# PhilippBongartz/RepeatResolver

Measured on AMD Instinct MI355X. Metric: sum-of-pairs DP cells/sec, higher is better.
Workload: dtype u32

## Files before the change

### repeatresolver_amd/csrc/pwr_device.hip

```cpp
#include <hip/hip_runtime.h>

#include <algorithm>
#include <chrono>
#include <cstdint>
#include <cstdio>
#include <cstdlib>
#include <cstring>
#include <new>
#include <thread>
#include <type_traits>
#include <vector>

#include "pwr.h"

#define PWR_INF 0x40000000u
#define PWR_BIG 0x7fffffff

struct Hdr {
    int W;
    int nslots;
    int nfree;
    int cur;
    int status;
    int stop;
// ... 593 lines not shown
            const unsigned upc = (y == 0 || y == W - 1) ? PWR_INF : max(w[5], covl);
            const int gq = (int)(carry + gin);
            rec2[2 * i] = make_int4((int)w[0] - gq, (int)w[1] - gq, (int)w[2] - gq, (int)w[3] - gq);
            rec2[2 * i + 1] = make_int4((int)(upc == PWR_INF ? PWR_INF - 1u : upc) - gq, gq, (int)PWR_INF - gq, 0);
            maxS = max(maxS, max(max(w[0], w[1]), max(max(w[2], w[3]), max(w[4], w[5]))));
        }
        carry += tot;
        __syncthreads();
    }
    const unsigned mx = (unsigned)(~block_min_u32<GATHER_NT>(~maxS, sh));
    for (int o = 32; o > 0; o >>= 1) ucost += __shfl_xor(ucost, o);
    if ((tid & 63) == 0) s_u[tid >> 6] = ucost;
    __syncthreads();
    if (tid == 0) {
        unsigned long long U = 0;
        for (int w = 0; w < GATHER_NT / 64; ++w) U += s_u[w];
        __hip_atomic_store(&part[g].ucost, U, __ATOMIC_RELAXED, __HIP_MEMORY_SCOPE_AGENT);
        __hip_atomic_store(&part[g].maxS, mx, __ATOMIC_RELAXED, __HIP_MEMORY_SCOPE_AGENT);
        __hip_atomic_store(&part[g].lastcov, tag, __ATOMIC_RELEASE, __HIP_MEMORY_SCOPE_AGENT);
    }
    if (g == GATHER_G - 1 && tid < 64) {
        unsigned long long Ut = 0, cs = 0;
        unsigned mxt = 0;
        if (tid < GATHER_G) {
            while (__hip_atomic_load(&part[tid].lastcov, __ATOMIC_ACQUIRE, __HIP_MEMORY_SCOPE_AGENT) != tag) __builtin_amdgcn_s_sleep(1);
            Ut = __hip_atomic_load(&part[tid].ucost, __ATOMIC_RELAXED, __HIP_MEMORY_SCOPE_AGENT);
            mxt = __hip_atomic_load(&part[tid].maxS, __ATOMIC_RELAXED, __HIP_MEMORY_SCOPE_AGENT);
            cs = part[tid].cells;
        }
        for (int o = 32; o > 0; o >>= 1) { Ut += __shfl_xor(Ut, o); cs += __shfl_xor(cs, o); mxt = max(mxt, (unsigned)__shfl_xor((int)mxt, o)); }
        if (tid == 0) {
            const unsigned long long bound = Ut + (unsigned long long)mxt * (unsigned long long)(2 * B + 4096);
            m->maxS = mxt; m->cells = cs;
            m->wide = (jb.force64 || !(bound < (unsigned long long)PWR_INF && carry < (1u << 29))) ? 1 : 0;
            if (m->wide) st.hdr->need64 = 65;
        }
    }
}

#define V2_D 128
#define V2_PD 512
#define V2_R 64
#define V2_SPINS 256
#define FBIG 0x3fffffff
#define UNI(v) __builtin_amdgcn_readfirstlane(v)

__device__ __forceinline__ unsigned acc_push(unsigned acc, unsigned long long mask)
{
    unsigned long long carry_out;
    asm("v_addc_co_u32_e64 %0, %1, %0, %0, %2" : "+v"(acc), "=s"(carry_out) : "s"(mask));
    return acc;
}
#define ICMP_SGE 39
#define ICMP_SLE 41

#define V2_LOAD(MSX, SLOT, AU, AG, AI, GL)                                                       \
    {                                                                                            \
        _Pragma("unroll") for (int i = 0; i < C; ++i) {                                          \
            const int y_ = lo + (MSX) * MS + lc + i;                                             \
            int4 p_ = make_int4(PWR_BIG / 2, PWR_BIG / 2, PWR_BIG / 2, PWR_BIG / 2);             \
            int4 q_ = make_int4(PWR_BIG / 2, 0, PWR_BIG / 2, 0);                                 \
            if (y_ <= hi) { p_ = rec2[2 * (y_ - lo)]; q_ = rec2[2 * (y_ - lo) + 1]; }            \
            ldsS[wave][SLOT][0][lc + i] = p_.x; ldsS[wave][SLOT][1][lc + i] = p_.y;              \
            ldsS[wave][SLOT][2][lc + i] = p_.z; ldsS[wave][SLOT][3][lc + i] = p_.w;              \
            AU[i] = q_.x; AG[i] = q_.y; AI[i] = q_.z;                                            \
        }                                                                                        \
        const int yq_ = lo + (MSX) * MS - 1;                                                     \
        GL = (yq_ >= lo && yq_ <= hi) ? UNI(rec2[2 * (yq_ - lo) + 1].y) : 0;                     \
    }

template <int NW, int C>
__global__ __launch_bounds__(NW * 64) void k_fill_v2(DState st, JobBufs jb)
{
    constexpr int MS = 64 * C, RS = NW * MS;
    constexpr int MBDUMP = NW * V2_D, PTDUMP = V2_PD;
    __shared__ unsigned long long mbQ[2 * (MBDUMP + NW * 64)];
    __shared__ unsigned long long ptQ[PTDUMP + NW * 64];
    __shared__ __attribute__((aligned(16))) int ldsS[NW][2][4][MS];
    __shared__ int rdone[NW];
    __shared__ int s_done;
#define LD64(REF) __hip_atomic_load(&(REF), __ATOMIC_RELAXED, __HIP_MEMORY_SCOPE_WORKGROUP)
#define LD32LO(REF) __hip_atomic_load((unsigned *)&(REF), __ATOMIC_RELAXED, __HIP_MEMORY_SCOPE_WORKGROUP)
#define ST64(REF, VAL, TAG) __hip_atomic_store(&(REF), ((unsigned long long)(unsigned)(TAG) << 32) | (unsigned)(VAL), __ATOMIC_RELAXED, __HIP_MEMORY_SCOPE_WORKGROUP)
#define MBP(W_, X_) mbQ[2 * ((W_) * V2_D + ((X_) & (V2_D - 1)))]
#define MBM(W_, X_) mbQ[2 * ((W_) * V2_D + ((X_) & (V2_D - 1))) + 1]
#define PTB(X_) ptQ[(X_) & (V2_PD - 1)]

    const int job = blockIdx.x, tid = threadIdx.x, lane = tid & 63;
    const int wave = UNI(tid >> 6);
    JobMeta *m = &jb.meta[job];
    const int L = UNI(m->L);
    if (jb.gate_v2 && st.hdr->fallback <= 0) return;
    if (!m->active || L <= 0 || !m->ok || m->wide || NOT_MINE(jb, job)) return;
    const unsigned long long t_clk0 = __builtin_amdgcn_s_memtime(), t_real0 = __builtin_amdgcn_s_memrealtime();
    for (int i = tid; i < 2 * (MBDUMP + NW * 64); i += NW * 64) mbQ[i] = 0;
    for (int i = tid; i < PTDUMP + NW * 64; i += NW * 64) ptQ[i] = 0;
    if (tid < NW) rdone[tid] = 0;
    if (tid == 0) s_done = 0;
    __syncthreads();

    const int lo = UNI(m->lo), hi = UNI(m->hi), W = UNI(m->W), B = st.B, H = st.H;
    const int *way = jb.way + (size_t)job * jb.Lmax;
    const uint8_t *seq = st.seq + st.rowoff[UNI(m->k)];
    const int4 *rec2 = jb.rec2 + (size_t)job * jb.colcap * 2;
    uint32_t *dirs = jb.dirs + (size_t)job * jb.dirstride;
    unsigned *lastM = jb.lastM + (size_t)job * jb.NC;
// ... 291 lines not shown
                    Mprev[i] = (rel0 + i < 0) ? PWR_INF : (unsigned)(gg[i] + p);
                }
            } else {
                unsigned Mn[C];
                unsigned fa = 0;
#pragma unroll
                for (int i = 0; i < C; ++i) {
                    fa |= (tg[i] >= p) ? (1u << i) : 0u;
                    p = min(p, tg[i]);
                    Mn[i] = (rel0 + i < 0) ? PWR_INF : (unsigned)(gg[i] + p);
                }
                const unsigned mrow = needP ? ePy : PWR_INF;
                const unsigned left0 = (unsigned)__builtin_amdgcn_update_dpp((int)mrow, (int)Mn[C - 1], DPP_WAVE_SHR1, 0xF, 0xF, false);
#pragma unroll
                for (int i = 0; i < C; ++i) {
                    const unsigned lf = i ? Mn[i > 0 ? i - 1 : 0] : left0;
                    const bool inb = (unsigned)(rel0 + i) < (unsigned)Bx;
                    accA[i] = (accA[i] << 1) | ((((fa >> i) & 1u) || (inb && Mn[i] == lf)) ? 1u : 0u);
                    lastM[wave * MS + lc + i] = inb ? Mn[i] : 0xffffffffu;
                    Mprev[i] = Mn[i];
                }
            }
            nacc = (x & 15) + 1;
            if (lane == 63) {
                ST64(MBP(wave, x), P_end, x + 1);
                ST64(MBM(wave, x), Mprev[C - 1], x + 1);
                if (ms == ms_hi) ST64(PTB(x), P_end, x + 1);
            }
            ran_prev = 1;
            V2_NEXT_ROW()
        }
        if (lane == 0) __hip_atomic_store(&rdone[wave], round + 1, __ATOMIC_RELAXED, __HIP_MEMORY_SCOPE_WORKGROUP);
        __syncthreads();
        if (UNI(__hip_atomic_load(&s_done, __ATOMIC_RELAXED, __HIP_MEMORY_SCOPE_WORKGROUP)) >= NW) break;
    }
    if (round >= max_rounds) {
        if (tid == 0) { m->ok = 0; atomicCAS(&st.hdr->status, 0, PWR_ERR_INTERNAL); }
        return;
    }
    if (tid == 0) {
        m->clk = (unsigned)(__builtin_amdgcn_s_memtime() - t_clk0);
        m->rclk = (unsigned)(__builtin_amdgcn_s_memrealtime() - t_real0);
        m->rounds = round;
        atomicAdd(&st.hdr->cells_computed, m->cells);
    }
#undef MBP
#undef MBM
#undef PTB
#undef LD64
#undef LD32LO
#undef ST64
}

#ifndef PWR_INTERIOR_CLS
#define PWR_INTERIOR_CLS 0
#endif
#define V3_TICKS() ((unsigned)(__builtin_amdgcn_s_memtime() >> 10))
#define V3_TIMEOUT_TICKS (1u << 19)
#define V4_RB 128

#ifdef PWR_DIAG
#define DG_DECL unsigned long long dg_wait_fast = 0, dg_wait_gen = 0, dg_wait_setup = 0, dg_t = 0, dg_t2 = 0, dg_cyc_int = 0, dg_cyc_gen16 = 0, dg_ts1 = 0, dg_ts2 = 0, dg_tl2 = 0; unsigned dg_log = 0; unsigned dg_int = 0, dg_gen16 = 0, dg_general = 0, dg_nowork = 0, dg_runs = 0, dg_switch = 0;
#define DG_T0() dg_t = __builtin_amdgcn_s_memtime();
#define DG_ADD(ACC) ACC += __builtin_amdgcn_s_memtime() - dg_t;
#define DG_INC(CNT, N) CNT += (N);
#define DG_T2() dg_t2 = __builtin_amdgcn_s_memtime();
#define DG_ADD2(ACC) ACC += __builtin_amdgcn_s_memtime() - dg_t2;
#else
#define DG_T2()
#define DG_ADD2(ACC)
#define DG_DECL
#define DG_T0()
#define DG_ADD(ACC)
#define DG_INC(CNT, N)
#endif
template <int NW, int C, bool WG1>
__global__ __launch_bounds__(WG1 ? NW * 64 : 128) void k_fill_v3(DState st, JobBufs jb)
{
    constexpr int MS = 64 * C, RS = NW * MS;
    constexpr int NL = WG1 ? NW : 1;
    constexpr int RB = WG1 ? 64 : V4_RB;
    __shared__ __attribute__((aligned(16))) int ldsS1[NL][2][4][MS];
    __shared__ unsigned long long rP[NL][RB];
    __shared__ int wprog[NL], wdone;
    const int vjob = WG1 ? (int)blockIdx.x : (int)(blockIdx.x + 8 * blockIdx.z), lane = threadIdx.x & 63;
    const int role = WG1 ? 0 : UNI((int)threadIdx.x >> 6);
    const int wave = WG1 ? UNI((int)threadIdx.x >> 6) : (int)blockIdx.y;
    const int lw = WG1 ? wave : 0, wr = WG1 ? (wave + 1) % NW : 0;
    if (vjob >= jb.njobs_launched * jb.smax) return;
    const int job = vjob / jb.smax;
    const SegDesc *const sd = jb.seg + (size_t)job * SEG_MAX + (vjob % jb.smax);
    JobMeta *m = &jb.meta[job];
    if (st.hdr->fallback > 0 && jb.v2_follows) return;
    if (!m->active || m->L <= 0 || !m->ok || m->wide || !sd->active || NOT_MINE(jb, job)) return;
    const int seg_xb = UNI(sd->xb), seg_fin = UNI(sd->fin);
    const int L = UNI(sd->xe) - seg_xb;
    const int Lf = seg_fin ? L - 1 : L;
    const int x_own = UNI(sd->xown) - seg_xb;
    const int g_own = x_own >> 4;
    const int chkA = x_own > 0 ? x_own : -1, chkB = seg_fin ? -1 : L;
    unsigned *const chk_w = jb.chk + (((size_t)job * (SEG_MAX + 1) + sd->s) * 2 + 0) * (size_t)jb.NC;
    unsigned *const chk_t = jb.chk + (((size_t)job * (SEG_MAX + 1) + sd->s + 1) * 2 + 1) * (size_t)jb.NC;
    const unsigned long long t_clk0 = __builtin_amdgcn_s_memtime(), t_real0 = __builtin_amdgcn_s_memrealtime();
    for (int i = threadIdx.x; i < NL * RB; i += blockDim.x) (&rP[0][0])[i] = 0;
    if (threadIdx.x < NL) wprog[threadIdx.x] = 0;
    if (threadIdx.x == 0) wdone = 0;
// ... 78 lines not shown
    int wcur = way[min(lane, L - 1)], scur = seq[min(lane, L - 1)];
    int wnxt = way[min(64 + lane, L - 1)], snxt = seq[min(64 + lane, L - 1)];
    const uint4 *desc = jb.desc + (size_t)job * jb.Lmax + seg_xb;
    const int fsh = 4 * (wave & 7);
    const unsigned *descw = (const unsigned *)desc + 1 + (wave >> 3);
    unsigned dca = desc[min(lane, L - 1)].x, dcf = descw[4 * min(lane, L - 1)] >> fsh;
    unsigned dna = desc[min(64 + lane, L - 1)].x, dnf = descw[4 * min(64 + lane, L - 1)];
    int a = max(0, __builtin_amdgcn_readlane(wcur, 0) - H), a_prev = 0, Bx_prev = 0;
    int sx = __builtin_amdgcn_readlane(scur, 0);

#define V4_CHK_STORE(XNEXT, AF, BEND)                                                            \
    if ((XNEXT) == chkA || (XNEXT) == chkB) {                                                    \
        unsigned *cv_ = (XNEXT) == chkA ? chk_w : chk_t;                                         \
        _Pragma("unroll") for (int i = 0; i < C; ++i) {                                          \
            const int y_ = lo + ms * MS + lc + i;                                                \
            cv_[wave * MS + lc + i] = (y_ >= (AF) && y_ < (BEND)) ? (unsigned)gg[i] + Mprev[i] : 0xffffffffu;    \
        }                                                                                        \
    }
#define V4_ALIGN_ACC(WANT)                                                                       \
    if (nacc != (WANT)) {                                                                        \
        const int sh_ = (WANT) - nacc;                                                           \
        _Pragma("unroll") for (int i = 0; i < C; ++i) { accA[i] <<= sh_; accC[i] <<= sh_; }      \
        nacc = (WANT);                                                                           \
    }
#define V4_FLUSH()                                                                               \
    if (gacc >= 0) {                                                                             \
        V4_ALIGN_ACC(16)                                                                         \
        uint32_t *d_ = dirs + (size_t)gacc * RS + (size_t)wave * MS + (size_t)lc;                \
        _Pragma("unroll") for (int i = 0; i < C; ++i) { if (gacc >= g_own) d_[i] = accA[i] | (accC[i] << 16); accA[i] = accC[i] = 0; } \
        gacc = -1; nacc = 0;                                                                     \
    }
#define V4_ROTATE_BLOCK()                                                                        \
    {                                                                                            \
        blk = x >> 6;                                                                            \
        wcur = wnxt; scur = snxt; dca = dna; dcf = dnf >> fsh;     \
        wnxt = way[min(x + 64 + lane, L - 1)];                                                   \
        snxt = seq[min(x + 64 + lane, L - 1)];                                                   \
        dna = desc[min(x + 64 + lane, L - 1)].x; dnf = descw[4 * min(x + 64 + lane, L - 1)];     \
    }
#define V4_NEXT_ROW()                                                                            \
    {                                                                                            \
        a_prev = a; Bx_prev = Bx;                                                                \
        ++x;                                                                                     \
        if (lane == 0) LST(wprog[lw], x);                                                            \
        if (x < L) {                                                                             \
            if ((x >> 6) != blk) V4_ROTATE_BLOCK()                                               \
            a = max(0, __builtin_amdgcn_readlane(wcur, x & 63) - H);                             \
            sx = __builtin_amdgcn_readlane(scur, x & 63);                                        \
        }                                                                                        \
    }

    DG_DECL
#ifdef PWR_DIAG
    unsigned long long *const tl = jb.diag + ((size_t)job * 32 + 31) * 4096 + (size_t)(sd->s * NW + wave) * 6;
    if (lane == 0 && sd->s * NW + wave < 680) { tl[0] = t_real0; tl[1] = __builtin_amdgcn_s_memrealtime(); tl[2] = 0; }
#endif
#define V4_EARLY_MASKS()                                                                         \
    if (early_hi >= (blk << 6)) {                                                                \
        const int b0_ = blk << 6;                                                                \
        const int lo_ = max(early_lo, b0_) - b0_, hi_ = min(early_hi, b0_ + 64) - b0_;           \
        const unsigned long long me_ = hi_ > lo_ ? ((hi_ - lo_ >= 64 ? ~0ull : ((1ull << (hi_ - lo_)) - 1ull)) << lo_) : 0ull; \
        const unsigned long long mf_ = early_hi < b0_ + 64 ? 1ull << (early_hi - b0_) : 0ull;    \
        bOm |= me_ | mf_; bMm |= me_ | mf_; bPm |= me_; bTm |= me_;                              \
    }
    bool dead = jb.stall_test && vjob == 0 && wave == 0;
    int first_pending = 0;
    int early_lo = 0, early_hi = -1;
    while (x < L && !dead) {
        ran_prev = UNI(ran_prev); gacc = UNI(gacc); nacc = UNI(nacc); blk = UNI(blk); ms = UNI(ms); cs = UNI(cs); gleft = UNI(gleft);
        x = UNI(x);
#ifdef PWR_DIAG
        if (ran_prev && !dg_tl2) { dg_tl2 = __builtin_amdgcn_s_memrealtime(); if (lane == 0 && sd->s * NW + wave < 680) { tl[2] = dg_tl2; tl[5] = (unsigned long long)x; } }
#endif
        if ((ran_prev || first_pending) && x < Lf) {
            unsigned long long bOm = __builtin_amdgcn_ballot_w64((dcf & 1u) != 0);
            const bool first = UNI(first_pending) != 0;
            if (first || ((bOm >> (x & 63)) & 1ull)) {
                first_pending = 0;
                unsigned long long bPm = __builtin_amdgcn_ballot_w64((dcf & 2u) != 0);
                unsigned long long bMm = __builtin_amdgcn_ballot_w64((dcf & 4u) != 0);
                unsigned long long bTm = __builtin_amdgcn_ballot_w64((dcf & 8u) != 0);
                if (first) { bOm |= 1ull << (x & 63); bMm |= 1ull << (x & 63); }
                V4_EARLY_MASKS()
                int dcaf = (int)(dca & 0xffffffu), dcb = min(dcaf + B, W);
                unsigned dcs = min(dca >> 24, 3u) * (unsigned)(MS * 4);
                if ((x >> 4) != gacc) { V4_FLUSH() gacc = x >> 4; }
                V4_ALIGN_ACC(x & 15)
                if (lane == 0) LST(wprog[lw], x);
                unsigned mlast_v = 0;
                if (first) {
                    const unsigned tagp = tagbase | (unsigned)x;
                    const int yq = lo + ms * MS - 1;
                    const bool needM = yq >= a_prev && yq < a_prev + Bx_prev;
                    unsigned long long eT = 0, eM = 0;
                    DG_T0()
#ifdef PWR_DIAG
                    const unsigned long long ev_t0 = __builtin_amdgcn_s_memrealtime();
#endif
                    const unsigned t0 = V3_TICKS();
                    for (unsigned spin = 1;; ++spin) {
                        eT = GLD(PTOT_PTR(a_prev, Bx_prev, x - 1));
                        eM = LLD(rP[lw][(x - 1) & (RB - 1)]);
                        if (UNI(TAGOF(eT)) == tagp && (!needM || UNI(TAGOF(eM)) == tagp)) break;
                        if ((spin & 1023u) == 0 && (V3_TICKS() - t0 > V3_TIMEOUT_TICKS || UNI(GLD(abortf)))) { dead = true; break; }
                        __builtin_amdgcn_s_sleep(1);
                    }
                    DG_ADD(dg_wait_gen)
#ifdef PWR_DIAG
                    if (lane == 0 && dg_general < 36) {
                        unsigned long long *ev = jb.diag + ((size_t)job * 32 + wave) * 4096 + 16 + 3 * dg_general;
                        ev[0] = (unsigned long long)x; ev[1] = ev_t0; ev[2] = __builtin_amdgcn_s_memrealtime();
                    }
#endif
                    DG_INC(dg_general, 1)
                    if (dead) break;
                    const int eTx = (int)UNI((unsigned)eT);
#pragma unroll
                    for (int i = 0; i < C; ++i) Mprev[i] = (unsigned)eTx;
                    mlast_v = yq < a_prev ? PWR_INF - (unsigned)gleft : (needM ? UNI((unsigned)eM) : (unsigned)eTx);
                    ran_prev = 1;
                } else if ((bMm >> (x & 63)) & 1ull) {
                    const unsigned tagp = tagbase | (unsigned)x;
                    unsigned long long w_ = LLD(rP[lw][(x - 1) & (RB - 1)]);
                    if (UNI(TAGOF(w_)) != tagp) {
                        DG_T0()
                        const unsigned t0 = V3_TICKS();
                        for (unsigned spin = 1;; ++spin) {
                            w_ = LLD(rP[lw][(x - 1) & (RB - 1)]);
                            if (UNI(TAGOF(w_)) == tagp) break;
                            if ((spin & 1023u) == 0 && (V3_TICKS() - t0 > V3_TIMEOUT_TICKS || UNI(GLD(abortf)))) { dead = true; break; }
                            __builtin_amdgcn_s_sleep(1);
                        }
                        DG_ADD(dg_wait_setup)
                        if (dead) break;
                    }
                    mlast_v = (unsigned)w_;
                }
                int ycol[C];
#pragma unroll
                for (int i = 0; i < C; ++i) ycol[i] = lo + ms * MS + lc + i;
                const char *const stab = (const char *)&ldsS1[lw][cs][0][lc];
                int sgr[C];
                {
                    const int *const srow0 = (const int *)(stab + __builtin_amdgcn_readlane((int)dcs, x & 63));
#pragma unroll
                    for (int i = 0; i < C; ++i) sgr[i] = srow0[i];
                }
                int af_done = a_prev;
                int g_af = 0, g_be = 0, g_cs = 0, g_cp = -1;
                DG_INC(dg_runs, 1)
                while (true) {
                    const int r_beg = x & 15, g0 = x - r_beg, r0 = g0 & 63;
                    int nrun = __builtin_ctz(~((unsigned)(bOm >> (r0 + r_beg)) & 0xffffu) | (1u << (16 - r_beg)));
                    nrun = min(nrun, Lf - x);
                    if (nrun <= 0) break;
                    const unsigned nPm = (unsigned)(bPm >> r0) & 0xffffu, kMm = (unsigned)(bMm >> r0) & 0xffffu, eTm = (unsigned)(bTm >> r0) & 0xffffu;
                    const unsigned p0 = (nPm >> r_beg) & 1u, m0 = (kMm >> r_beg) & 1u, t0_ = (eTm >> r_beg) & 1u;
                    const unsigned diff = ((nPm ^ (0u - p0)) | (kMm ^ (0u - m0)) | ((p0 & m0) ? 0u : (eTm ^ (0u - t0_)))) & 0xffffu;
                    const int nsame = __builtin_ctz((diff >> r_beg) | 0x10000u);
                    const bool mixed16 = r_beg == 0 && nrun == 16 && nsame < 16;
                    const int r_e = mixed16 ? 16 : r_beg + min(nrun, nsame);
                    const unsigned et_here = (eTm >> r_beg) & ((1u << (r_e - r_beg)) - 1u);
                    const int cls = mixed16 ? 3 : ((p0 & m0) ? (et_here ? 1 : 0) : ((p0 | m0 | t0_) == 0u ? 2 : 3));
                    if (gacc < 0) gacc = x >> 4;
#ifdef PWR_DIAG
                    if (!dg_ts1 && x >= 1024) dg_ts1 = __builtin_amdgcn_s_memrealtime();
                    if (!dg_ts2 && x >= 2048) dg_ts2 = __builtin_amdgcn_s_memrealtime();
#endif
                    if (WG1) {
                        const int need = g0 + 16 - RB + 2;
                        if (need > 0 && UNI(LLD(wprog[wr])) < need) {
                            DG_T0()
                            const unsigned t0 = V3_TICKS();
                            for (unsigned spin = 1;; ++spin) {
                                if (UNI(LLD(wprog[wr])) >= need) break;
                                if ((spin & 1023u) == 0 && (V3_TICKS() - t0 > V3_TIMEOUT_TICKS || UNI(GLD(abortf)))) { dead = true; break; }
                                __builtin_amdgcn_s_sleep(1);
                            }
                            DG_ADD(dg_wait_setup)
                            if (dead) break;
                        }
                    }
                    unsigned long long *const gq0 = gmy + (size_t)g0;
                    const unsigned tag_g0 = tagbase | (unsigned)g0;
                    const unsigned long long *const ringP = &rP[lw][g0 & (RB - 1)];
                    if (g0 != g_cp) {
                        const int src = 4 * min(r0 + lane, 63);
                        g_af = __builtin_amdgcn_ds_bpermute(src, dcaf);
                        g_be = __builtin_amdgcn_ds_bpermute(src, dcb);
                        g_cs = __builtin_amdgcn_ds_bpermute(src, (int)dcs);
                        g_cp = g0;
                    }
                    auto group_row = [&](const int r, auto cls_, auto bits_) __attribute__((always_inline)) {
                        constexpr int CLS = decltype(cls_)::value;
                        constexpr bool BITS = decltype(bits_)::value;
                        bool bP = CLS <= 1 || CLS == 4, bM = CLS <= 1 || CLS == 4;
                        if (CLS == 3) { bP = (nPm >> r) & 1u; bM = (kMm >> r) & 1u; }
                        int af = 0, bend = 0;
                        if (CLS >= 2) af = __builtin_amdgcn_readlane(g_af, r);
                        if (CLS == 1 || CLS == 3 || CLS == 4) bend = __builtin_amdgcn_readlane(g_be, r);
                        const int Mleft_v = bM ? (int)mlast_v : (int)PWR_INF - gleft;
                        const int pm1_0 = __builtin_amdgcn_update_dpp(Mleft_v, (int)Mprev[C - 1], DPP_WAVE_SHR1, 0xF, 0xF, false);
                        int tg[C];
                        int run = FBIG;
#pragma unroll
                        for (int i = 0; i < C; ++i) {
                            const int pm1 = i ? (int)Mprev[i > 0 ? i - 1 : 0] : pm1_0;
                            const int d = pm1 + sgr[i];
                            const int u = (int)Mprev[i] + ug[i];
                            if (BITS) accC[i] = acc_push(accC[i], __builtin_amdgcn_sicmp(d, u, ICMP_SLE));
                            const int t3 = min(min(d, u), ig[i]);
                            bool inb = true;
                            if (CLS == 1 || CLS == 4) inb = ycol[i] < bend;
                            if (CLS == 2) inb = ycol[i] >= af;
                            if (CLS == 3) inb = (unsigned)(ycol[i] - af) < (unsigned)(bend - af);
                            tg[i] = inb ? t3 : FBIG;
                            run = min(run, tg[i]);
                        }
                        unsigned long long fP = 0;
                        if (CLS != 2) fP = LLD(ringP[r]);
                        __builtin_amdgcn_sched_barrier(0);
#define V4_SCAN_STEP(CTRL, RMASK) { const int t_ = __builtin_amdgcn_update_dpp(PWR_BIG, incl, CTRL, RMASK, 0xF, false); incl = min(incl, t_); }
#define V4_FENCE() __builtin_amdgcn_sched_barrier(0)
                        int incl = run;
                        V4_SCAN_STEP(DPP_ROW_SHR(1), 0xF) V4_FENCE();
                        const int soff = __builtin_amdgcn_readlane(g_cs, r + 1);
                        V4_FENCE(); V4_SCAN_STEP(DPP_ROW_SHR(2), 0xF) V4_FENCE();
                        const int *const srow = (const int *)(stab + soff);
                        V4_FENCE(); V4_SCAN_STEP(DPP_ROW_SHR(4), 0xF) V4_FENCE();
#pragma unroll
                        for (int i = 0; i < C; ++i) sgr[i] = srow[i];
                        V4_FENCE(); V4_SCAN_STEP(DPP_ROW_SHR(8), 0xF) V4_FENCE();
                        const unsigned tagx = tag_g0 + (unsigned)(r + 1);
                        V4_FENCE(); V4_SCAN_STEP(DPP_ROW_BCAST15, 0xA) V4_FENCE();
                        V4_FENCE(); V4_SCAN_STEP(DPP_ROW_BCAST31, 0xC) V4_FENCE();
#undef V4_SCAN_STEP
#undef V4_FENCE
                        if (bP && __builtin_expect(UNI(TAGOF(fP)) != tagx, 0)) {
                            DG_T0()
                            const unsigned t0 = V3_TICKS();
                            for (unsigned spin = 1; !dead; ++spin) {
                                fP = LLD(ringP[r]);
                                if (UNI(TAGOF(fP)) == tagx) break;
                                if ((spin & 1023u) == 0 && (V3_TICKS() - t0 > V3_TIMEOUT_TICKS || UNI(GLD(abortf)))) { dead = true; break; }
                                __builtin_amdgcn_s_sleep(1);
                            }
                            DG_ADD(dg_wait_fast)
                        }
                        const int P_in_v = bP ? (int)(unsigned)fP : PWR_BIG;
                        const int P_end_v = min(P_in_v, incl);
                        const int pq = min(P_in_v, FBIG);
                        int p = min(__builtin_amdgcn_update_dpp(pq, incl, DPP_WAVE_SHR1, 0xF, 0xF, false), pq);
#pragma unroll
                        for (int i = 0; i < C; ++i) {
                            if (BITS) accA[i] = acc_push(accA[i], __builtin_amdgcn_sicmp(tg[i], p, ICMP_SGE));
                            p = min(p, tg[i]);
                            Mprev[i] = (unsigned)(CLS == 0 ? p : min(p, ig[i]));
                        }
                        mlast_v = (unsigned)fP;
                        if (lane == 63) {
                            if (WG1) {
                                GST2(gq0 + r, P_end_v, tagx);
                                LST(rP[wr][(g0 + r) & (RB - 1)], ((unsigned long long)tagx << 32) | (unsigned)P_end_v);
                            } else {
                                typedef unsigned v2u_ __attribute__((ext_vector_type(2)));
                                v2u_ w2_; w2_.x = (unsigned)P_end_v; w2_.y = tagx;
                                asm volatile("global_store_dwordx2 %0, %1, %2 sc1" :: "v"(8 * r), "v"(w2_), "s"(gq0) : "memory");
                            }
                        }
                    };
                    int r_end = r_e;
                    DG_T2()
                    using WithBits = std::integral_constant<bool, true>;
                    using NoBits = std::integral_constant<bool, false>;
                    const bool warmup = (x >> 4) < g_own;
                    if (warmup && r_beg == 0 && r_e == 16 && cls != 3) {
                        if (cls == 0) {
#pragma unroll
                            for (int r = 0; r < 16; ++r) group_row(r, std::integral_constant<int, PWR_INTERIOR_CLS>{}, NoBits{});
                            DG_INC(dg_int, 16)
                            DG_ADD2(dg_cyc_int)
                        } else if (cls == 1) {
#pragma unroll
                            for (int r = 0; r < 16; ++r) group_row(r, std::integral_constant<int, 1>{}, NoBits{});
                        } else {
#pragma unroll
                            for (int r = 0; r < 16; ++r) group_row(r, std::integral_constant<int, 2>{}, NoBits{});
                        }
                    } else if (cls == 0 && r_beg == 0 && r_e == 16) {
#pragma unroll
                        for (int r = 0; r < 16; ++r) group_row(r, std::integral_constant<int, PWR_INTERIOR_CLS>{}, WithBits{});
                        DG_INC(dg_int, 16)
                        DG_ADD2(dg_cyc_int)
                    } else if (cls == 1 && r_beg == 0 && r_e == 16) {
#pragma unroll
                        for (int r = 0; r < 16; ++r) group_row(r, std::integral_constant<int, 1>{}, WithBits{});
                    } else if (cls == 3 && r_beg == 0 && r_e == 16) {
#pragma unroll
                        for (int r = 0; r < 16; ++r) group_row(r, std::integral_constant<int, 3>{}, WithBits{});
                    } else if (cls == 2 && r_beg == 0 && r_e == 16) {
#pragma unroll
                        for (int r = 0; r < 16; ++r) group_row(r, std::integral_constant<int, 2>{}, WithBits{});
                    } else {
                        int r = r_beg;
                        for (; r < r_end && (r & 3) && !dead; ++r) group_row(r, std::integral_constant<int, 3>{}, WithBits{});
#define V4_BLOCKS(K) for (; r + 4 <= r_end && !dead; r += 4) { group_row(r, std::integral_constant<int, K>{}, WithBits{}); group_row(r + 1, std::integral_constant<int, K>{}, WithBits{}); \
                                                               group_row(r + 2, std::integral_constant<int, K>{}, WithBits{}); group_row(r + 3, std::integral_constant<int, K>{}, WithBits{}); }
                        if (cls == 0) V4_BLOCKS(0)
                        else if (cls == 1) V4_BLOCKS(1)
                        else if (cls == 2) V4_BLOCKS(2)
#undef V4_BLOCKS
                        for (; r < r_end && !dead; ++r) group_row(r, std::integral_constant<int, 3>{}, WithBits{});
                        r_end = r;
                    }
                    if (!(cls == 0 && r_beg == 0 && r_e == 16)) { DG_INC(dg_gen16, r_end - r_beg) DG_ADD2(dg_cyc_gen16) }
                    x = g0 + r_end;
#ifdef PWR_DIAG
                    if (lane == 0 && dg_log < 1270) {
                        unsigned long long *lg = jb.diag + ((size_t)job * 32 + wave) * 4096 + 256 + 3 * dg_log;
                        lg[0] = (unsigned long long)x | ((unsigned long long)cls << 32) | ((unsigned long long)(r_end - r_beg) << 40); lg[1] = __builtin_amdgcn_s_memrealtime();
                        lg[2] = dg_wait_fast + dg_wait_gen + dg_wait_setup;
                    }
                    dg_log += 1;
#endif
                    af_done = __builtin_amdgcn_readlane(dcaf, (x - 1) & 63);
                    if ((x & 15) == 0) {
                        uint32_t *d_ = dirs + (size_t)gacc * RS + (size_t)wave * MS + (size_t)lc;
#pragma unroll
                        for (int i = 0; i < C; ++i) { if (gacc >= g_own) d_[i] = accA[i] | (accC[i] << 16); accA[i] = accC[i] = 0; }
                        gacc = -1; nacc = 0;
                        V4_CHK_STORE(x, af_done, min(af_done + B, W))
                    } else nacc = x & 15;
                    if (dead || x >= Lf) break;
                    if ((x >> 6) != blk) {
                        V4_ROTATE_BLOCK()
                        bOm = __builtin_amdgcn_ballot_w64((dcf & 1u) != 0); bPm = __builtin_amdgcn_ballot_w64((dcf & 2u) != 0);
                        bMm = __builtin_amdgcn_ballot_w64((dcf & 4u) != 0); bTm = __builtin_amdgcn_ballot_w64((dcf & 8u) != 0);
                        V4_EARLY_MASKS()
                        dcaf = (int)(dca & 0xffffffu); dcb = min(dcaf + B, W);
                        dcs = min(dca >> 24, 3u) * (unsigned)(MS * 4);
                        g_cp = -1;
                        const int *const srow0 = (const int *)(stab + __builtin_amdgcn_readlane((int)dcs, 0));
#pragma unroll
                        for (int i = 0; i < C; ++i) sgr[i] = srow0[i];
                    }
                    if (lane == 0) LST(wprog[lw], x);
                }
                a_prev = af_done; Bx_prev = min(B, W - af_done);
                if (dead) break;
                if (x < L) {
                    if ((x >> 6) != blk) V4_ROTATE_BLOCK()
                    a = max(0, __builtin_amdgcn_readlane(wcur, x & 63) - H);
                    sx = __builtin_amdgcn_readlane(scur, x & 63);
                }
                if (lane == 0) LST(wprog[lw], x);
                continue;
            }
        }
        if (dead || x >= L) break;

        x = UNI(x); ms = UNI(ms); msn = UNI(msn); a = UNI(a); a_prev = UNI(a_prev); Bx_prev = UNI(Bx_prev);
        sx = UNI(sx); gacc = UNI(gacc); nacc = UNI(nacc); blk = UNI(blk); gleft = UNI(gleft); gleftn = UNI(gleftn); ran_prev = UNI(ran_prev); cs = UNI(cs);
        const int Bx = min(B, W - a);
        const int ms_lo = (a - lo) / MS, ms_hi = (a + Bx - 1 - lo) / MS;
        if (ms < ms_lo) {
            ms += NW;
            if (ms == msn) {
#pragma unroll
                for (int i = 0; i < C; ++i) { ug[i] = nu[i]; gg[i] = ng[i]; ig[i] = ni[i]; }
                gleft = gleftn;
                cs ^= 1;
            } else {
                while (ms < ms_lo) ms += NW;
// ... 20 lines not shown
                if (xs < 1) xs = xn;
                const int an = __builtin_amdgcn_readlane(anf_l, xn & 63);
                if (ms < (an - lo) / MS) { xs = xn; first_pending = 0; }
                else { early_lo = xs; early_hi = xn; first_pending = xs > 0 ? 1 : 0; }
            }
            DG_INC(dg_nowork, xs - x)
            if (xs > x) {
                const int al = __builtin_amdgcn_readlane((int)dca, (xs - 1) & 63) & 0xffffff;
                a_prev = al; Bx_prev = min(B, W - al);
            }
            x = xs;
            ran_prev = 0;
            if (lane == 0) LST(wprog[lw], x);
            if (x < L) {
                if ((x >> 6) != blk) V4_ROTATE_BLOCK()
                a = max(0, __builtin_amdgcn_readlane(wcur, x & 63) - H);
                sx = __builtin_amdgcn_readlane(scur, x & 63);
            }
            continue;
        }
        if (!ran_prev && x > 0 && x < Lf) { first_pending = 1; continue; }
        const int y0 = lo + ms * MS;
        const int yq = y0 - 1;
        const bool needP = ms > ms_lo;
        const bool needM = x > 0 && yq >= a_prev && yq < a_prev + Bx_prev;
        const bool needT = x > 0 && ((yq >= a_prev + Bx_prev) || !ran_prev);
        unsigned ePx = 0, ePy = 0, eMy = 0, eTx = 0;
        if (WG1 && x - RB + 2 > 0) {
            const unsigned t0 = V3_TICKS();
            for (unsigned spin = 1; UNI(LLD(wprog[wr])) < x - RB + 2; ++spin) {
                if ((spin & 1023u) == 0 && (V3_TICKS() - t0 > V3_TIMEOUT_TICKS || UNI(GLD(abortf)))) { dead = true; break; }
                __builtin_amdgcn_s_sleep(1);
            }
            if (dead) break;
        }
        {
            const unsigned tagx = tagbase | (unsigned)(x + 1), tagp = tagbase | (unsigned)x;
#ifdef PWR_DIAG
            const unsigned long long ev_t0 = __builtin_amdgcn_s_memrealtime();
#endif
            DG_T0()
            const unsigned t0 = V3_TICKS();
            for (unsigned spin = 1;; ++spin) {
                const unsigned long long eP = LLD(rP[lw][x & (RB - 1)]);
                const unsigned long long eM = LLD(rP[lw][(x - 1) & (RB - 1)]), eT = needT ? GLD(PTOT_PTR(a_prev, Bx_prev, x - 1)) : 0ull;
                ePx = UNI((unsigned)eP); ePy = ePx; eMy = UNI((unsigned)eM); eTx = UNI((unsigned)eT);
                const bool ready = (!needP || UNI(TAGOF(eP)) == tagx) &&
                                   (!needM || UNI(TAGOF(eM)) == tagp) && (!needT || UNI(TAGOF(eT)) == tagp);
                if (ready) break;
                if ((spin & 1023u) == 0 && (V3_TICKS() - t0 > V3_TIMEOUT_TICKS || UNI(GLD(abortf)))) { dead = true; break; }
                __builtin_amdgcn_s_sleep(1);
            }
#ifdef PWR_DIAG
            if (lane == 0 && dg_general < 36) {
                unsigned long long *ev = jb.diag + ((size_t)job * 32 + wave) * 4096 + 16 + 3 * dg_general;
                ev[0] = (unsigned long long)x; ev[1] = ev_t0; ev[2] = __builtin_amdgcn_s_memrealtime();
            }
#endif
            DG_ADD(dg_wait_gen)
            DG_INC(dg_general, 1)
            if (dead) break;
        }
        int Mleft = (int)PWR_INF;
        if (x == 0) Mleft = (src_c < 0 || yq == src_c) ? -gleft : (int)PWR_INF - gleft;
        else if (yq < a_prev) Mleft = (int)PWR_INF - gleft;
        else if (needM) Mleft = (int)eMy;
        else Mleft = (int)eTx;
        const int P_in = needP ? (int)ePx : PWR_BIG;
        if (x > 0 && !ran_prev) {
#pragma unroll
            for (int i = 0; i < C; ++i) Mprev[i] = eTx;
        }
        if ((x >> 4) != gacc) { V4_FLUSH() gacc = x >> 4; }
        V4_ALIGN_ACC(x & 15)
        const int pm1_0 = __builtin_amdgcn_update_dpp(Mleft, (int)Mprev[C - 1], DPP_WAVE_SHR1, 0xF, 0xF, false);
        const int sxc = min(max(sx, 0), 3);
        const int rel0 = y0 + lc - a;
        int tg[C];
        int run = PWR_BIG;
#pragma unroll
        for (int i = 0; i < C; ++i) {
            const int pm1 = i ? (int)Mprev[i > 0 ? i - 1 : 0] : pm1_0;
            const int d = pm1 + ldsS1[lw][cs][sxc][lc + i];
            const int u = (int)Mprev[i] + ug[i];
            accC[i] = (accC[i] << 1) | ((d <= u) ? 1u : 0u);
            const int t3 = min(min(d, u), ig[i]);
            tg[i] = ((unsigned)(rel0 + i) < (unsigned)Bx) ? t3 : PWR_BIG;
            run = min(run, tg[i]);
        }
        const int incl = wave_incl_min(run);
        const int excl = __builtin_amdgcn_update_dpp(PWR_BIG, incl, DPP_WAVE_SHR1, 0xF, 0xF, false);
        const int P_end = min(P_in, __builtin_amdgcn_readlane(incl, 63));
        int p = min(P_in, excl);
        if (x != Lf) {
#pragma unroll
            for (int i = 0; i < C; ++i) {
                accA[i] = (accA[i] << 1) | ((tg[i] >= p) ? 1u : 0u);
                p = min(p, tg[i]);
                Mprev[i] = (unsigned)((rel0 + i < 0) ? ig[i] : p);
            }
        } else {
            unsigned Mn[C];
            unsigned fa = 0;
#pragma unroll
            for (int i = 0; i < C; ++i) {
                fa |= (tg[i] >= p) ? (1u << i) : 0u;
                p = min(p, tg[i]);
                Mn[i] = (rel0 + i < 0) ? PWR_INF : (unsigned)(gg[i] + p);
                Mprev[i] = (unsigned)((rel0 + i < 0) ? ig[i] : p);
            }
            const unsigned mrow = needP ? (unsigned)gleft + ePy : PWR_INF;
            const unsigned left0 = (unsigned)__builtin_amdgcn_update_dpp((int)mrow, (int)Mn[C - 1], DPP_WAVE_SHR1, 0xF, 0xF, false);
#pragma unroll
            for (int i = 0; i < C; ++i) {
                const unsigned lf = i ? Mn[i > 0 ? i - 1 : 0] : left0;
                const bool inb = (unsigned)(rel0 + i) < (unsigned)Bx;
                accA[i] = (accA[i] << 1) | ((((fa >> i) & 1u) || (inb && Mn[i] == lf)) ? 1u : 0u);
                lastM[wave * MS + lc + i] = inb ? Mn[i] : 0xffffffffu;
            }
        }
        nacc = (x & 15) + 1;
        if (lane == 63) {
            GST(gmy + (size_t)x, P_end, x);
            if (WG1) LST(rP[wr][x & (RB - 1)], ((unsigned long long)(tagbase | (unsigned)(x + 1)) << 32) | (unsigned)P_end);
        }
        ran_prev = 1;
        V4_CHK_STORE(x + 1, a, a + Bx)
        V4_NEXT_ROW()
    }
    V4_FLUSH()
#ifdef PWR_DIAG
    if (lane == 0) {
        unsigned long long *dgp = jb.diag + ((size_t)job * 32 + wave) * 4096;
        dgp[0] = __builtin_amdgcn_s_memtime() - t_clk0; dgp[1] = dg_wait_fast; dgp[2] = dg_wait_gen; dgp[3] = dg_wait_setup;
        dgp[4] = ((unsigned long long)dg_int << 32) | dg_gen16; dgp[5] = ((unsigned long long)dg_general << 32) | dg_nowork;
        dgp[6] = ((unsigned long long)dg_runs << 32) | dg_switch; dgp[7] = (unsigned long long)L;
        dgp[12] = dg_log; dgp[8] = dg_cyc_gen16; dgp[9] = dg_ts1; dgp[10] = dg_ts2; dgp[11] = dg_cyc_int;
    }
#endif
#ifdef PWR_DIAG
    if (lane == 0 && sd->s * NW + wave < 680) { tl[3] = __builtin_amdgcn_s_memrealtime(); tl[4] = (unsigned long long)L | ((unsigned long long)(dg_wait_fast + dg_wait_gen + dg_wait_setup) << 20); }
#endif
    if (lane == 0) { LST(wprog[lw], 0x7fffffff); LST(wdone, 1); }
    if (dead) {
        if (lane == 0) __hip_atomic_store(abortf, 1, __ATOMIC_RELAXED, __HIP_MEMORY_SCOPE_AGENT);
        return;
    }
    if (wave == 0 && lane == 0) {
        if (sd->s == 0) {
            m->clk = (unsigned)(__builtin_amdgcn_s_memtime() - t_clk0);
            m->rclk = (unsigned)(__builtin_amdgcn_s_memrealtime() - t_real0);
            m->rounds = 0;
        }
        atomicAdd(&st.hdr->cells_computed, sd->cells);
    }
#undef V4_CHK_STORE
#undef V4_EARLY_MASKS
#undef PTOT_PTR
#undef GLD
#undef GST
#undef GST2
#undef TAGOF
#undef LLD
#undef LST
#undef V4_LOADS
#undef V4_ALIGN_ACC
#undef V4_FLUSH
#undef V4_ROTATE_BLOCK
#undef V4_NEXT_ROW
}

__device__ __forceinline__ bool seg_check_applies(const DState &st, const JobBufs &jb, int job, const JobMeta *m)
{
    return m->active && m->L > 0 && m->ok && !m->wide && !m->abort && !(st.hdr->fallback > 0 && jb.v2_follows) && !NOT_MINE(jb, job) && m->nseg > 1;
}

__device__ __forceinline__ void seg_check_body(const DState &st, const JobBufs &jb, const int job, const int s, const int tid)
{
    __shared__ int s_min[4], s_max[4], s_bad;
    JobMeta *m = &jb.meta[job];
    if (!seg_check_applies(st, jb, job, m)) return;
    if (s >= m->nseg) return;
    const SegDesc *sd = jb.seg + (size_t)job * SEG_MAX + s;
    const int xr = sd->xown - 1;
    const int lo = m->lo, W = m->W, B = st.B, H = st.H, RS = jb.NC;
// ... 2961 lines not shown
```

Measured before the change: 57.53 billion.

## Interleave independent per-row work into DPP scan latency gaps and precompute band guards

Fills the stall slots between the dependent DPP prefix-min scan steps in the per-row group kernel with independent work: the ring load, the next row's score offset and edge readlanes, the substitution-row loads, the traceback compare/accumulate pushes, and the next row's band guard masks. Band-membership tests for the edge classes are now computed one row ahead as lane masks and applied with inverse_ballot, instead of being compared inline. This aims to hide the cross-lane DPP latency on the serial row dependency chain, at the cost of extra registers and fragile scheduling fences. Diagnostic logging is also restricted to a single segment.

```diff
diff --git a/repeatresolver_amd/csrc/pwr_device.hip b/repeatresolver_amd/csrc/pwr_device.hip
--- a/repeatresolver_amd/csrc/pwr_device.hip
+++ b/repeatresolver_amd/csrc/pwr_device.hip
@@ -669,6 +669,7 @@
     return acc;
 }
 #define ICMP_SGE 39
+#define ICMP_SLT 40
 #define ICMP_SLE 41
 
 #define V2_LOAD(MSX, SLOT, AU, AG, AI, GL)                                                       \
@@ -1066,6 +1067,9 @@
 #undef ST64
 }
 
+#ifndef PWR_DIAG_SEG
+#define PWR_DIAG_SEG 0
+#endif
 #ifndef PWR_INTERIOR_CLS
 #define PWR_INTERIOR_CLS 0
 #endif
@@ -1250,6 +1254,7 @@
 
     DG_DECL
 #ifdef PWR_DIAG
+    const bool dg_me = sd->s == min(PWR_DIAG_SEG, UNI(m->nseg) - 1);
     unsigned long long *const tl = jb.diag + ((size_t)job * 32 + 31) * 4096 + (size_t)(sd->s * NW + wave) * 6;
     if (lane == 0 && sd->s * NW + wave < 680) { tl[0] = t_real0; tl[1] = __builtin_amdgcn_s_memrealtime(); tl[2] = 0; }
 #endif
@@ -1305,7 +1310,7 @@
                     }
                     DG_ADD(dg_wait_gen)
 #ifdef PWR_DIAG
-                    if (lane == 0 && dg_general < 36) {
+                    if (lane == 0 && dg_me && dg_general < 36) {
                         unsigned long long *ev = jb.diag + ((size_t)job * 32 + wave) * 4096 + 16 + 3 * dg_general;
                         ev[0] = (unsigned long long)x; ev[1] = ev_t0; ev[2] = __builtin_amdgcn_s_memrealtime();
                     }
@@ -1389,49 +1394,106 @@
                         g_cs = __builtin_amdgcn_ds_bpermute(src, (int)dcs);
                         g_cp = g0;
                     }
+                    unsigned long long gd[C];
+#pragma unroll
+                    for (int i = 0; i < C; ++i) gd[i] = ~0ull;
+                    auto guard_head = [&](const int r, auto cls_) __attribute__((always_inline)) {
+                        constexpr int CLS = decltype(cls_)::value;
+                        if (CLS == 1 || CLS == 2 || CLS == 4) {
+                            const int e_ = __builtin_amdgcn_readlane(CLS == 2 ? g_af : g_be, r);
+#pragma unroll
+                            for (int i = 0; i < C; ++i) gd[i] = __builtin_amdgcn_sicmp(ycol[i], e_, CLS == 2 ? ICMP_SGE : ICMP_SLT);
+                        }
+                    };
                     auto group_row = [&](const int r, auto cls_, auto bits_) __attribute__((always_inline)) {
                         constexpr int CLS = decltype(cls_)::value;
                         constexpr bool BITS = decltype(bits_)::value;
+                        constexpr bool AHEAD = CLS == 1 || CLS == 2 || CLS == 4;
+                        constexpr int CH = (C + 1) / 2;
                         bool bP = CLS <= 1 || CLS == 4, bM = CLS <= 1 || CLS == 4;
                         if (CLS == 3) { bP = (nPm >> r) & 1u; bM = (kMm >> r) & 1u; }
                         int af = 0, bend = 0;
-                        if (CLS >= 2) af = __builtin_amdgcn_readlane(g_af, r);
-                        if (CLS == 1 || CLS == 3 || CLS == 4) bend = __builtin_amdgcn_readlane(g_be, r);
+                        if (CLS == 3) { af = __builtin_amdgcn_readlane(g_af, r); bend = __builtin_amdgcn_readlane(g_be, r); }
                         const int Mleft_v = bM ? (int)mlast_v : (int)PWR_INF - gleft;
                         const int pm1_0 = __builtin_amdgcn_update_dpp(Mleft_v, (int)Mprev[C - 1], DPP_WAVE_SHR1, 0xF, 0xF, false);
-                        int tg[C];
+                        int tg[C], dq[C], uq[C];
                         int run = FBIG;
 #pragma unroll
                         for (int i = 0; i < C; ++i) {
                             const int pm1 = i ? (int)Mprev[i > 0 ? i - 1 : 0] : pm1_0;
                             const int d = pm1 + sgr[i];
                             const int u = (int)Mprev[i] + ug[i];
-                            if (BITS) accC[i] = acc_push(accC[i], __builtin_amdgcn_sicmp(d, u, ICMP_SLE));
+                            dq[i] = d; uq[i] = u;
                             const int t3 = min(min(d, u), ig[i]);
                             bool inb = true;
-                            if (CLS == 1 || CLS == 4) inb = ycol[i] < bend;
-                            if (CLS == 2) inb = ycol[i] >= af;
+                            if (AHEAD) inb = __builtin_amdgcn_inverse_ballot_w64(gd[i]);
                             if (CLS == 3) inb = (unsigned)(ycol[i] - af) < (unsigned)(bend - af);
                             tg[i] = inb ? t3 : FBIG;
                             run = min(run, tg[i]);
                         }
-                        unsigned long long fP = 0;
-                        if (CLS != 2) fP = LLD(ringP[r]);
-                        __builtin_amdgcn_sched_barrier(0);
+                        unsigned long long fP = 0, cm[C];
+                        unsigned tagx = 0;
+                        int gb = 0, soff = 0;
+                        const int *srow = nullptr;
 #define V4_SCAN_STEP(CTRL, RMASK) { const int t_ = __builtin_amdgcn_update_dpp(PWR_BIG, incl, CTRL, RMASK, 0xF, false); incl = min(incl, t_); }
 #define V4_FENCE() __builtin_amdgcn_sched_barrier(0)
+#define V4_F_RING() { fP = LLD(ringP[r]); V4_FENCE(); }
+#define V4_F_SOFF() { soff = __builtin_amdgcn_readlane(g_cs, r + 1); V4_FENCE(); }
+#define V4_F_EDGE() { if (AHEAD) { gb = __builtin_amdgcn_readlane(CLS == 2 ? g_af : g_be, r + 1); V4_FENCE(); } }
+#define V4_F_TAG()  { tagx = tag_g0 + (unsigned)(r + 1); if (CLS == 2) asm volatile("" :: "s"(tagx)); V4_FENCE(); }
+#define V4_F_SROW() { srow = (const int *)(stab + soff); V4_FENCE(); }
+#define V4_F_SGR(LO, HI) { _Pragma("unroll") for (int i = 0; i < C; ++i) if (i >= (LO) && i < (HI)) sgr[i] = srow[i]; V4_FENCE(); }
+#define V4_F_CC(I)  { if ((I) < C) { cm[(I) < C ? (I) : 0] = __builtin_amdgcn_sicmp(dq[(I) < C ? (I) : 0], uq[(I) < C ? (I) : 0], ICMP_SLE); V4_FENCE(); } }
+#define V4_F_CP(I)  { if ((I) < C) { accC[(I) < C ? (I) : 0] = acc_push(accC[(I) < C ? (I) : 0], cm[(I) < C ? (I) : 0]); V4_FENCE(); } }
+#define V4_F_GD(I)  { if (AHEAD && (I) < C) { gd[(I) < C ? (I) : 0] = __builtin_amdgcn_sicmp(ycol[(I) < C ? (I) : 0], gb, CLS == 2 ? ICMP_SGE : ICMP_SLT); V4_FENCE(); } }
+#define V4_F_BIG()  { asm volatile("" : "+v"(big)); V4_FENCE(); }
+                        int big = PWR_BIG;
+                        auto gap = [&](auto k_) __attribute__((always_inline)) {
+                            constexpr int K = decltype(k_)::value + (CLS == 2 ? 1 : 0);
+                            if constexpr (decltype(k_)::value == 5 && CLS != 2) V4_F_BIG()
+                            if constexpr (K == 0) V4_F_RING()
+                            if constexpr (!BITS && AHEAD) {
+                                if constexpr (K == 1) { V4_F_SOFF() V4_F_EDGE() }
+                                if constexpr (K == 2) { V4_F_SROW() V4_F_TAG() }
+                                if constexpr (K == 3) { V4_F_SGR(0, CH) V4_F_SGR(CH, C) }
+                                if constexpr (K == 4) { _Pragma("unroll") for (int i = 0; i < CH; ++i) V4_F_GD(i) }
+                                if constexpr (K == 5) { _Pragma("unroll") for (int i = CH; i < C; ++i) V4_F_GD(i) }
+                            }
+                            if constexpr (!BITS && !AHEAD) {
+                                if constexpr (K == 1) { V4_F_SOFF() V4_F_TAG() }
+                                if constexpr (K == 2) { V4_F_SROW() V4_F_SGR(0, CH) }
+                                if constexpr (K == 3) { V4_F_SGR(CH, C) }
+                            }
+                            if constexpr (BITS) {
+                                if constexpr (K == 1) { V4_F_SOFF() V4_F_EDGE() }
+                                if constexpr (K == 2) { V4_F_SROW() V4_F_SGR(0, CH) }
+                                if constexpr (K == 3) { _Pragma("unroll") for (int i = 0; i < C - 1; ++i) V4_F_CC(i) }
+                                if constexpr (K == 4) { V4_F_CC(C - 1) _Pragma("unroll") for (int i = 0; i < CH; ++i) { V4_F_CP(i) if (i == 0) V4_F_SGR(CH, C) } }
+                                if constexpr (K == 5) { _Pragma("unroll") for (int i = CH; i < C; ++i) { V4_F_CP(i) if (i == CH) { V4_F_TAG() V4_F_GD(0) } } if (CH == C) { V4_F_TAG() V4_F_GD(0) } }
+                                if constexpr (K == 6) { _Pragma("unroll") for (int i = 1; i < CH; ++i) V4_F_GD(i) }
+                                if constexpr (K == 7) { _Pragma("unroll") for (int i = CH; i < C; ++i) V4_F_GD(i) }
+                            }
+                        };
+                        using std::integral_constant;
                         int incl = run;
-                        V4_SCAN_STEP(DPP_ROW_SHR(1), 0xF) V4_FENCE();
-                        const int soff = __builtin_amdgcn_readlane(g_cs, r + 1);
-                        V4_FENCE(); V4_SCAN_STEP(DPP_ROW_SHR(2), 0xF) V4_FENCE();
-                        const int *const srow = (const int *)(stab + soff);
-                        V4_FENCE(); V4_SCAN_STEP(DPP_ROW_SHR(4), 0xF) V4_FENCE();
-#pragma unroll
-                        for (int i = 0; i < C; ++i) sgr[i] = srow[i];
-                        V4_FENCE(); V4_SCAN_STEP(DPP_ROW_SHR(8), 0xF) V4_FENCE();
-                        const unsigned tagx = tag_g0 + (unsigned)(r + 1);
-                        V4_FENCE(); V4_SCAN_STEP(DPP_ROW_BCAST15, 0xA) V4_FENCE();
-                        V4_FENCE(); V4_SCAN_STEP(DPP_ROW_BCAST31, 0xC) V4_FENCE();
+                        V4_FENCE(); gap(integral_constant<int, 0>{}); V4_SCAN_STEP(DPP_ROW_SHR(1), 0xF) V4_FENCE();
+                        gap(integral_constant<int, 1>{}); V4_SCAN_STEP(DPP_ROW_SHR(2), 0xF) V4_FENCE();
+                        gap(integral_constant<int, 2>{}); V4_SCAN_STEP(DPP_ROW_SHR(4), 0xF) V4_FENCE();
+                        gap(integral_constant<int, 3>{}); V4_SCAN_STEP(DPP_ROW_SHR(8), 0xF) V4_FENCE();
+                        gap(integral_constant<int, 4>{}); V4_SCAN_STEP(DPP_ROW_BCAST15, 0xA) V4_FENCE();
+                        gap(integral_constant<int, 5>{});
+                        { const int t_ = __builtin_amdgcn_update_dpp(big, incl, DPP_ROW_BCAST31, 0xC, 0xF, false); incl = min(incl, t_); } V4_FENCE();
+                        gap(integral_constant<int, 6>{}); gap(integral_constant<int, 7>{});
+#undef V4_F_BIG
+#undef V4_F_RING
+#undef V4_F_SOFF
+#undef V4_F_EDGE
+#undef V4_F_TAG
+#undef V4_F_SROW
+#undef V4_F_SGR
+#undef V4_F_CC
+#undef V4_F_CP
+#undef V4_F_GD
 #undef V4_SCAN_STEP
 #undef V4_FENCE
                         if (bP && __builtin_expect(UNI(TAGOF(fP)) != tagx, 0)) {
@@ -1448,6 +1510,9 @@
                         const int P_in_v = bP ? (int)(unsigned)fP : PWR_BIG;
                         const int P_end_v = min(P_in_v, incl);
                         const int pq = min(P_in_v, FBIG);
+                        typedef unsigned v2u_ __attribute__((ext_vector_type(2)));
+                        v2u_ w2_; w2_.x = (unsigned)P_end_v; w2_.y = tagx;
+                        if (!WG1 && CLS != 2) asm volatile("" : "+v"(w2_));
                         int p = min(__builtin_amdgcn_update_dpp(pq, incl, DPP_WAVE_SHR1, 0xF, 0xF, false), pq);
 #pragma unroll
                         for (int i = 0; i < C; ++i) {
@@ -1461,8 +1526,6 @@
                                 GST2(gq0 + r, P_end_v, tagx);
                                 LST(rP[wr][(g0 + r) & (RB - 1)], ((unsigned long long)tagx << 32) | (unsigned)P_end_v);
                             } else {
-                                typedef unsigned v2u_ __attribute__((ext_vector_type(2)));
-                                v2u_ w2_; w2_.x = (unsigned)P_end_v; w2_.y = tagx;
                                 asm volatile("global_store_dwordx2 %0, %1, %2 sc1" :: "v"(8 * r), "v"(w2_), "s"(gq0) : "memory");
                             }
                         }
@@ -1474,39 +1537,45 @@
                     const bool warmup = (x >> 4) < g_own;
                     if (warmup && r_beg == 0 && r_e == 16 && cls != 3) {
                         if (cls == 0) {
+                            guard_head(0, std::integral_constant<int, PWR_INTERIOR_CLS>{});
 #pragma unroll
                             for (int r = 0; r < 16; ++r) group_row(r, std::integral_constant<int, PWR_INTERIOR_CLS>{}, NoBits{});
                             DG_INC(dg_int, 16)
                             DG_ADD2(dg_cyc_int)
                         } else if (cls == 1) {
+                            guard_head(0, std::integral_constant<int, 1>{});
 #pragma unroll
                             for (int r = 0; r < 16; ++r) group_row(r, std::integral_constant<int, 1>{}, NoBits{});
                         } else {
+                            guard_head(0, std::integral_constant<int, 2>{});
 #pragma unroll
                             for (int r = 0; r < 16; ++r) group_row(r, std::integral_constant<int, 2>{}, NoBits{});
                         }
                     } else if (cls == 0 && r_beg == 0 && r_e == 16) {
+                        guard_head(0, std::integral_constant<int, PWR_INTERIOR_CLS>{});
 #pragma unroll
                         for (int r = 0; r < 16; ++r) group_row(r, std::integral_constant<int, PWR_INTERIOR_CLS>{}, WithBits{});
                         DG_INC(dg_int, 16)
                         DG_ADD2(dg_cyc_int)
                     } else if (cls == 1 && r_beg == 0 && r_e == 16) {
+                        guard_head(0, std::integral_constant<int, 1>{});
 #pragma unroll
                         for (int r = 0; r < 16; ++r) group_row(r, std::integral_constant<int, 1>{}, WithBits{});
                     } else if (cls == 3 && r_beg == 0 && r_e == 16) {
 #pragma unroll
                         for (int r = 0; r < 16; ++r) group_row(r, std::integral_constant<int, 3>{}, WithBits{});
                     } else if (cls == 2 && r_beg == 0 && r_e == 16) {
+                        guard_head(0, std::integral_constant<int, 2>{});
 #pragma unroll
                         for (int r = 0; r < 16; ++r) group_row(r, std::integral_constant<int, 2>{}, WithBits{});
                     } else {
                         int r = r_beg;
                         for (; r < r_end && (r & 3) && !dead; ++r) group_row(r, std::integral_constant<int, 3>{}, WithBits{});
-#define V4_BLOCKS(K) for (; r + 4 <= r_end && !dead; r += 4) { group_row(r, std::integral_constant<int, K>{}, WithBits{}); group_row(r + 1, std::integral_constant<int, K>{}, WithBits{}); \
+#define V4_BLOCKS(K) guard_head(r, std::integral_constant<int, K>{}); for (; r + 4 <= r_end && !dead; r += 4) { group_row(r, std::integral_constant<int, K>{}, WithBits{}); group_row(r + 1, std::integral_constant<int, K>{}, WithBits{}); \
                                                                group_row(r + 2, std::integral_constant<int, K>{}, WithBits{}); group_row(r + 3, std::integral_constant<int, K>{}, WithBits{}); }
-                        if (cls == 0) V4_BLOCKS(0)
-                        else if (cls == 1) V4_BLOCKS(1)
-                        else if (cls == 2) V4_BLOCKS(2)
+                        if (cls == 0) { V4_BLOCKS(0) }
+                        else if (cls == 1) { V4_BLOCKS(1) }
+                        else if (cls == 2) { V4_BLOCKS(2) }
 #undef V4_BLOCKS
                         for (; r < r_end && !dead; ++r) group_row(r, std::integral_constant<int, 3>{}, WithBits{});
                         r_end = r;
@@ -1514,9 +1583,9 @@
                     if (!(cls == 0 && r_beg == 0 && r_e == 16)) { DG_INC(dg_gen16, r_end - r_beg) DG_ADD2(dg_cyc_gen16) }
                     x = g0 + r_end;
 #ifdef PWR_DIAG
-                    if (lane == 0 && dg_log < 1270) {
+                    if (lane == 0 && dg_me && dg_log < 1270) {
                         unsigned long long *lg = jb.diag + ((size_t)job * 32 + wave) * 4096 + 256 + 3 * dg_log;
-                        lg[0] = (unsigned long long)x | ((unsigned long long)cls << 32) | ((unsigned long long)(r_end - r_beg) << 40); lg[1] = __builtin_amdgcn_s_memrealtime();
+                        lg[0] = (unsigned long long)x | ((unsigned long long)(cls | (warmup ? 16 : 0)) << 32) | ((unsigned long long)(r_end - r_beg) << 40); lg[1] = __builtin_amdgcn_s_memrealtime();
                         lg[2] = dg_wait_fast + dg_wait_gen + dg_wait_setup;
                     }
                     dg_log += 1;
@@ -1643,7 +1712,7 @@
                 __builtin_amdgcn_s_sleep(1);
             }
 #ifdef PWR_DIAG
-            if (lane == 0 && dg_general < 36) {
+            if (lane == 0 && dg_me && dg_general < 36) {
                 unsigned long long *ev = jb.diag + ((size_t)job * 32 + wave) * 4096 + 16 + 3 * dg_general;
                 ev[0] = (unsigned long long)x; ev[1] = ev_t0; ev[2] = __builtin_amdgcn_s_memrealtime();
             }
@@ -1721,7 +1790,7 @@
     }
     V4_FLUSH()
 #ifdef PWR_DIAG
-    if (lane == 0) {
+    if (lane == 0 && dg_me) {
         unsigned long long *dgp = jb.diag + ((size_t)job * 32 + wave) * 4096;
         dgp[0] = __builtin_amdgcn_s_memtime() - t_clk0; dgp[1] = dg_wait_fast; dgp[2] = dg_wait_gen; dgp[3] = dg_wait_setup;
         dgp[4] = ((unsigned long long)dg_int << 32) | dg_gen16; dgp[5] = ((unsigned long long)dg_general << 32) | dg_nowork;
```

After: 58.67 billion (median of 6 runs). 2.0% higher.
